# aymenboudhina/Multimodal_VQVAE_compression_audio_tactile

Measured on AMD Instinct MI355X. Metric: encode+VQ+decode token-frames/sec (1 frame = 13.33 ms of paired 24 kHz audio+tactile), higher is better.
Workload: dtype f32

## Files before the change

include/mvq.h:

```cpp
#ifndef MVQ_H
#define MVQ_H

#include <stddef.h>
#include <stdint.h>

#ifdef __cplusplus
extern "C" {
#endif

#define MVQ_OK 0
#define MVQ_EINVAL (-1)
#define MVQ_EUNSUPPORTED (-2)
#define MVQ_EHIP (-3)

#define MVQ_ACT_NONE 0
#define MVQ_ACT_TANH 1
#define MVQ_ACT_GELU 2

int mvq_abi_version(void);
const char* mvq_last_error(void);
unsigned mvq_build_flags(void);

typedef struct mvq_profile_entry {
    char kernel[96];
// ... 305 lines not shown
int mvq_encoder_stream_fwd_f32(const mvq_stack* s, float* state, const int32_t* slots, int n_group, int n_slots, const float* x_new, int n,
                               long long samples_before, int last, float* z, int z_len, void* workspace, size_t workspace_bytes, void* stream);
int mvq_decoder_out_len(const mvq_stack* s, int t);
size_t mvq_decoder_workspace_bytes(const mvq_stack* s, int batch, int t);
int mvq_decoder_fwd_f32(const mvq_stack* s, const float* z, float* y, void* workspace, size_t workspace_bytes, int batch, int t, void* stream);
int mvq_decoder_stream_plan(const mvq_stack* s, int tokens_before, int n, int last, int32_t* stages, int stages_cap, int32_t* emit);
size_t mvq_decoder_stream_state_floats(const mvq_stack* s);
size_t mvq_decoder_stream_workspace_bytes(const mvq_stack* s, int n_group, int tokens_before, int n, int last);
int mvq_decoder_stream_fwd_f32(const mvq_stack* s, float* state, const int32_t* slots, int n_group, int n_slots, const float* z_new, int n,
                               int tokens_before, int last, float* y, int y_len, void* workspace, size_t workspace_bytes, void* stream);
size_t mvq_decoder_saved_bytes(const mvq_stack* s, int batch, int t);
int mvq_decoder_fwd_saving_f32(const mvq_stack* s, const float* z, float* y, void* saved, size_t saved_bytes, void* workspace, size_t workspace_bytes,
                               int batch, int t, void* stream);
int mvq_decoder_bwd_input_f32(const mvq_stack* s, const void* saved, size_t saved_bytes, const float* gy, float* gz, void* workspace,
                              size_t workspace_bytes, int batch, int t, void* stream);

typedef struct mvq_ar_args {
    int batch, t_lat, t_audio, tactile_only, books_use, rvq_k, c_lat, c_ff, code_dim, heads, chunk;
    float ln_eps, tok_eps, scale;
    const float *zt, *k_all, *v_all, *pe;
    const float *lnq_g, *lnq_b, *wq, *wo, *lnf_g, *lnf_b, *w1, *b1, *w3, *b3;
    const float *tok_g, *tok_b, *wd, *bd, *wu, *bu, *books;
    float *z_run, *r_tokens;
    int32_t* idx_out;
} mvq_ar_args;
size_t mvq_ar_workspace_bytes(int batch, int t_lat);
int mvq_ar_latents_f32(const mvq_ar_args* args, void* workspace, size_t workspace_bytes, void* stream);
int mvq_ar_latents_staged_f32(const mvq_ar_args* args, void* workspace, size_t workspace_bytes, void* stream);
int mvq_ar_latents_staged_carry_f32(const mvq_ar_args* args, const float* z_prev, float* z_last_out, void* workspace,
                                    size_t workspace_bytes, void* stream);
int mvq_ar_latents_staged_rate_f32(const mvq_ar_args* args, int packet_tok, int min_books, int mode, float tol2, int budget,
                                   const float* z_prev, float* z_last_out, uint8_t* nb_valid_out, uint8_t* nb_sent_out, void* workspace,
                                   size_t workspace_bytes, void* stream);
int mvq_ar_check(const void* workspace, void* stream);

#ifdef __cplusplus
}
#endif
#endif
```

multimodal_vqvae_compression_audio_tactile_amd/_lib.py:

```python
from __future__ import annotations

import ctypes
import subprocess
from ctypes import c_char_p, c_float, c_int, c_size_t, c_void_p
from pathlib import Path

_PKG = Path(__file__).resolve().parent
import os as _os
SO_PATH = Path(_os.environ["MVQ_LIB_PATH"]).resolve() if _os.environ.get("MVQ_LIB_PATH") else _PKG / "libmvq_hip.so"
_lib = None

class EncoderDesc(ctypes.Structure):
    _fields_ = [("d_model", c_int), ("n_strides", c_int), ("strides", c_int * 8), ("d_latent", c_int)]


class DecoderDesc(ctypes.Structure):
    _fields_ = [("input_channel", c_int), ("channels", c_int), ("n_rates", c_int), ("rates", c_int * 8), ("d_out", c_int), ("output_padding", c_int)]


class ArArgs(ctypes.Structure):
    _fields_ = ([(n, c_int) for n in ("batch", "t_lat", "t_audio", "tactile_only", "books_use", "rvq_k", "c_lat", "c_ff", "code_dim", "heads", "chunk")]
                + [(n, c_float) for n in ("ln_eps", "tok_eps", "scale")]
                + [(n, c_void_p) for n in ("zt", "k_all", "v_all", "pe", "lnq_g", "lnq_b", "wq", "wo", "lnf_g", "lnf_b", "w1", "b1", "w3", "b3",
                                           "tok_g", "tok_b", "wd", "bd", "wu", "bu", "books", "z_run", "r_tokens", "idx_out")])
# ... 123 lines not shown
    "mvq_sub3d_f32": (c_int, [c_void_p, c_size_t, c_size_t] * 3 + [c_int] * 3 + [c_void_p]),
    "mvq_copy3d_f32": (c_int, [c_void_p, c_size_t, c_size_t] * 2 + [c_int] * 3 + [c_void_p]),
    "mvq_encoder_create": (c_int, [ctypes.POINTER(c_void_p), ctypes.POINTER(EncoderDesc), ctypes.POINTER(c_void_p), c_void_p, c_size_t, c_void_p]),
    "mvq_decoder_create": (c_int, [ctypes.POINTER(c_void_p), ctypes.POINTER(DecoderDesc), ctypes.POINTER(c_void_p), c_void_p, c_size_t, c_void_p]),
    "mvq_stack_destroy": (None, [c_void_p]),
    "mvq_stack_param_count": (c_int, [c_void_p]),
    "mvq_stack_param_info": (c_int, [c_void_p, c_int, c_char_p, c_int, ctypes.POINTER(c_int)]),
    "mvq_stack_weights_bytes": (c_size_t, [c_void_p]),
    "mvq_stack_set_plan": (c_int, [c_void_p, c_int, c_int]),
    "mvq_encoder_out_len": (c_int, [c_void_p, c_int]),
    "mvq_encoder_workspace_bytes": (c_size_t, [c_void_p, c_int, c_int]),
    "mvq_encoder_fwd_f32": (c_int, [c_void_p, c_void_p, c_void_p, c_void_p, c_size_t, c_int, c_int, c_void_p]),
    "mvq_decoder_out_len": (c_int, [c_void_p, c_int]),
    "mvq_decoder_workspace_bytes": (c_size_t, [c_void_p, c_int, c_int]),
    "mvq_decoder_fwd_f32": (c_int, [c_void_p, c_void_p, c_void_p, c_void_p, c_size_t, c_int, c_int, c_void_p]),
    "mvq_encoder_stream_plan": (c_int, [c_void_p, ctypes.c_longlong, c_int, c_int, c_void_p, c_int, c_void_p]),
    "mvq_encoder_stream_state_floats": (c_size_t, [c_void_p]),
    "mvq_encoder_stream_workspace_bytes": (c_size_t, [c_void_p, c_int, ctypes.c_longlong, c_int, c_int]),
    "mvq_encoder_stream_fwd_f32": (c_int, [c_void_p, c_void_p, c_void_p, c_int, c_int, c_void_p, c_int, ctypes.c_longlong, c_int, c_void_p, c_int,
                                           c_void_p, c_size_t, c_void_p]),
    "mvq_decoder_stream_plan":(c_int, [c_void_p, c_int, c_int, c_int, c_void_p, c_int, c_void_p]),
    "mvq_decoder_stream_state_floats": (c_size_t, [c_void_p]),
    "mvq_decoder_stream_workspace_bytes": (c_size_t, [c_void_p] + [c_int] * 4),
    "mvq_decoder_stream_fwd_f32": (c_int, [c_void_p, c_void_p, c_void_p, c_int, c_int, c_void_p, c_int, c_int, c_int, c_void_p, c_int, c_void_p,
                                           c_size_t, c_void_p]),
    "mvq_decoder_saved_bytes": (c_size_t, [c_void_p, c_int, c_int]),
    "mvq_decoder_fwd_saving_f32": (c_int, [c_void_p, c_void_p, c_void_p, c_void_p, c_size_t, c_void_p, c_size_t, c_int, c_int, c_void_p]),
    "mvq_decoder_bwd_input_f32": (c_int, [c_void_p, c_void_p, c_size_t, c_void_p, c_void_p, c_void_p, c_size_t, c_int, c_int, c_void_p]),
    "mvq_ar_workspace_bytes": (c_size_t, [c_int, c_int]),
    "mvq_ar_latents_f32": (c_int, [ctypes.POINTER(ArArgs), c_void_p, c_size_t, c_void_p]),
    "mvq_ar_latents_staged_f32": (c_int, [ctypes.POINTER(ArArgs), c_void_p, c_size_t, c_void_p]),
    "mvq_ar_latents_staged_carry_f32": (c_int, [ctypes.POINTER(ArArgs), c_void_p, c_void_p, c_void_p, c_size_t, c_void_p]),
    "mvq_ar_latents_staged_rate_f32": (c_int, [ctypes.POINTER(ArArgs)] + [c_int] * 3 + [c_float, c_int] + [c_void_p] * 5 + [c_size_t, c_void_p]),
    "mvq_ar_check": (c_int, [c_void_p, c_void_p]),
}


class MvqError(RuntimeError):
    """Raised when a libmvq_hip entry point returns a negative status."""


def build(force: bool = False) -> Path:
    args = ["make", "-C", str(_PKG / "csrc"), "-j8"]
    if force:
        args.append("-B")
    res = subprocess.run(args, capture_output=True, text=True)
    if res.returncode != 0:
        raise RuntimeError("building libmvq_hip.so failed:\n" + res.stdout[-4000:] + res.stderr[-4000:])
    return SO_PATH


def lib():
    global _lib
    if _lib is None:
        if not SO_PATH.exists():
            raise MvqError(f"{SO_PATH} is missing: run `python -c 'import __graft_entry__ as g; g.build()'` "
                           "(there is no CPU fallback for the MI355X path)")
        handle = ctypes.CDLL(str(SO_PATH))
        for name, (res, args) in EXPORTS.items():
            fn = getattr(handle, name)
            fn.restype = res
            fn.argtypes = args
        flags = int(handle.mvq_build_flags())
        if flags & 0xFFFF and _os.environ.get("MVQ_ALLOW_TIMING_BUILD") != "1":
            raise MvqError(f"{SO_PATH}: mvq_build_flags() = {flags:#x} (MVQ_NO_DMA in the environment; include/mvq.h).  "
                           "Only A/B runs may load it: set MVQ_ALLOW_TIMING_BUILD=1 to do so.")
# ... 15 lines not shown
```

multimodal_vqvae_compression_audio_tactile_amd/csrc/ar_fused.hip:

```cpp
#include <hip/hip_runtime.h>
#include <stdint.h>
#include <stdio.h>
#include <stdlib.h>
#include "../../include/mvq.h"
#include "conv_dispatch.hpp"
#include "conv_lat.hpp"
#include "kernels_small.hpp"
#include "det_math.hpp"
#include "ln_lat.hpp"

namespace mvq {
void set_last_error(const char* msg);
hipError_t launch_layernorm_lat_io(const LnIo& io, int B, int C, int n, hipStream_t s);

namespace {

constexpr int NTHR = 512;
constexpr int C_LAT = 1024, C_FF = 2048, D_CODE = 96, HEADS = 8, DH = C_LAT / HEADS, CHUNK = 16;

struct ArK {
    mvq_ar_args a;
    float *q16, *qT, *Q16, *ctx16, *y1T, *hdn16, *h16, *zpT, *rN16, *rD16, *qD16;
    unsigned* bar;
    int nblocks;
// ... 307 lines not shown
    if (!a.tactile_only) {
        {
            LnIo& io = tab[0].ln; tab[0].type = ST_LN; tab[0].adv = ADV_LN_PREV | ADV_LN_Y1;
            io.x = nullptr; io.prev = a.z_run; io.prev_sb = cT; io.prev_sc = (size_t)Tl;
            io.pe = a.pe; io.gamma = a.lnq_g; io.beta = a.lnq_b; io.eps = a.ln_eps; io.post_scale = 1.0f;
            io.y0 = k.q16; io.y0_sb = c16; io.y0_sc = p16;
            io.y1 = k.qT; io.y1_sb = cT; io.y1_sc = (size_t)Tl;
        }
        gemm(1, ST_GEMM64, k.q16, C_LAT, a.wq, nullptr, C_LAT, nullptr, 0, k.Q16, CHUNK, 0);
        tab[2].type = ST_ATTN;
        gemm(3, ST_GEMM64, k.ctx16, C_LAT, a.wo, nullptr, C_LAT, k.qT, 0, k.y1T, Tl, ADV_RES | ADV_Y);
        {
            LnIo& io = tab[4].ln; tab[4].type = ST_LN; tab[4].adv = ADV_LN_X;
            io.x = k.y1T; io.x_sb = cT; io.x_sc = (size_t)Tl;
            io.gamma = a.lnf_g; io.beta = a.lnf_b; io.eps = a.ln_eps; io.post_scale = 1.0f;
            io.y0 = k.hdn16; io.y0_sb = c16; io.y0_sc = p16;
        }
        gemm(5, ST_GEMM64, k.hdn16, C_LAT, a.w1, a.b1, C_FF, nullptr, MVQ_ACT_GELU, k.h16, CHUNK, 0);
        gemm(6, ST_GEMM64, k.h16, C_FF, a.w3, a.b3, C_LAT, k.y1T, 0, k.zpT, Tl, ADV_RES | ADV_Y);
        zpred = k.zpT;
    }
    {
        LnIo& io = tab[7].ln; tab[7].type = ST_LN; tab[7].adv = ADV_LN_X | ADV_LN_SUB;
        io.x = a.zt; io.x_sb = cT; io.x_sc = (size_t)Tl;
        io.sub = zpred; io.sub_sb = cT; io.sub_sc = (size_t)Tl;
        io.gamma = a.tok_g; io.beta = a.tok_b; io.eps = a.tok_eps; io.post_scale = a.scale; io.do_tanh = 1;
        io.y0 = k.rN16; io.y0_sb = c16; io.y0_sc = p16;
    }
    gemm(8, ST_GEMM64, k.rN16, C_LAT, a.wd, a.bd, D_CODE, nullptr, 0, k.rD16, CHUNK, 0);
    tab[9].type = ST_RVQ;
    gemm(10, ST_GEMM32, k.qD16, D_CODE, a.wu, a.bu, C_LAT, zpred, 0, a.z_run, Tl, ADV_RES | ADV_Y);
}

}
}

extern "C" {

size_t mvq_ar_workspace_bytes(int batch, int t_lat)
{
    if (batch <= 0 || t_lat <= 0) return 0;
    const size_t c = mvq::C_LAT, p = mvq::CHUNK;
    const size_t f16 = (size_t)batch * p, fT = (size_t)batch * t_lat;
    const size_t floats = c * f16 * 5  + (size_t)mvq::C_FF * f16 + 2 * (size_t)mvq::D_CODE * f16 + c * fT * 3 ;
    return floats * sizeof(float) + 256  + 256 ;
}

static int ar_prepare(const mvq_ar_args* args, void* workspace, size_t workspace_bytes, mvq::ArKT& kt, bool& done)
{
    using namespace mvq;
    auto fail = [](int code, const char* msg) { set_last_error(msg); return code; };
    done = false;
    if (!args) return fail(MVQ_EINVAL, "ar_latents: null argument");
    const mvq_ar_args& a = *args;
    if (a.batch < 0 || a.t_lat < 0 || a.t_audio < 0 || a.books_use < 0) return fail(MVQ_EINVAL, "ar_latents: bad shape");
    if (a.batch == 0 || a.t_lat == 0) { done = true; return MVQ_OK; }
    if (a.c_lat != C_LAT || a.c_ff != C_FF || a.code_dim != D_CODE || a.heads != HEADS || a.chunk != CHUNK)
        return fail(MVQ_EUNSUPPORTED, "ar_latents: the fused loop covers the reference's shapes (c_lat 1024, FFN 2048, 8 heads, code dim 96, chunks of 16)");
    if (a.rvq_k <= 0 || a.rvq_k > 512) return fail(MVQ_EUNSUPPORTED, "ar_latents: K <= 512 codes per book");
    if (!a.zt || !a.z_run || !a.tok_g || !a.tok_b || !a.wd || !a.bd || !a.wu || !a.bu || (a.books_use > 0 && !a.books) || !workspace)
        return fail(MVQ_EINVAL, "ar_latents: null tensor");
    if (!a.tactile_only && (!a.pe || !a.lnq_g || !a.lnq_b || !a.wq || !a.wo || !a.lnf_g || !a.lnf_b || !a.w1 || !a.b1 || !a.w3 || !a.b3 ||
                            (a.t_audio > 0 && (!a.k_all || !a.v_all))))
        return fail(MVQ_EINVAL, "ar_latents: null predictor tensor");
    if (workspace_bytes < mvq_ar_workspace_bytes(a.batch, a.t_lat)) return fail(MVQ_EINVAL, "ar_latents: workspace too small (mvq_ar_workspace_bytes)");
    if ((reinterpret_cast<uintptr_t>(a.books) & 15) != 0) return fail(MVQ_EINVAL, "ar_latents: books must be 16-byte aligned");
    if (conv_mpad(C_LAT) != C_LAT || conv_mpad(C_FF) != C_FF || conv_mpad(D_CODE) != D_CODE) return fail(MVQ_EUNSUPPORTED, "ar_latents: packed-row padding");

    kt = ArKT{};
    ArK& k = kt.k;
    k.a = a;
    char* p = reinterpret_cast<char*>(workspace);
    p += (256 - reinterpret_cast<uintptr_t>(p) % 256) % 256;
    k.bar = reinterpret_cast<unsigned*>(p); p += 256;
    auto take = [&](size_t floats) { float* q = reinterpret_cast<float*>(p); p += floats * sizeof(float); return q; };
    const size_t f16 = (size_t)a.batch * CHUNK, fT = (size_t)a.batch * a.t_lat;
    k.q16 = take(C_LAT * f16); k.Q16 = take(C_LAT * f16); k.ctx16 = take(C_LAT * f16); k.hdn16 = take(C_LAT * f16); k.rN16 = take(C_LAT * f16);
    k.h16 = take((size_t)C_FF * f16); k.rD16 = take((size_t)D_CODE * f16); k.qD16 = take((size_t)D_CODE * f16);
// ... 125 lines not shown
                                             reinterpret_cast<float*>(a.idx_out) + s, (size_t)Tl, 0, a.books_use * B, 1, n, st);
                    if (e == hipSuccess && a.r_tokens)
                        e = launch_strided3d(k.rD16, (size_t)D_CODE * CHUNK, CHUNK, nullptr, 0, 0, a.r_tokens + s, (size_t)D_CODE * Tl, (size_t)Tl, B, D_CODE, n, st);
                    break;
                }
            }
        }
    }
    if (e == hipSuccess && z_last_out)
        e = launch_strided3d(a.z_run + (Tl - 1), (size_t)C_LAT * Tl, (size_t)Tl, nullptr, 0, 0, z_last_out, C_LAT, 1, B, C_LAT, 1, st);
    if (e != hipSuccess) return fail(MVQ_EHIP, hipGetErrorString(e));
    return MVQ_OK;
}

int mvq_ar_latents_staged_f32(const mvq_ar_args* args, void* workspace, size_t workspace_bytes, void* stream)
{
    return ar_staged(args, nullptr, nullptr, workspace, workspace_bytes, stream);
}

int mvq_ar_latents_staged_carry_f32(const mvq_ar_args* args, const float* z_prev, float* z_last_out, void* workspace,
                                    size_t workspace_bytes, void* stream)
{
    return ar_staged(args, z_prev, z_last_out, workspace, workspace_bytes, stream);
}

int mvq_ar_latents_staged_rate_f32(const mvq_ar_args* args, int packet_tok, int min_books, int mode, float tol2, int budget,
                                   const float* z_prev, float* z_last_out, uint8_t* nb_valid_out, uint8_t* nb_sent_out, void* workspace,
                                   size_t workspace_bytes, void* stream)
{
    const ArRate r{packet_tok, min_books, mode, budget, tol2, nb_valid_out, nb_sent_out};
    return ar_staged(args, z_prev, z_last_out, workspace, workspace_bytes, stream, &r);
}

int mvq_ar_check(const void* workspace, void* stream)
{
    if (!workspace) return MVQ_EINVAL;
    const char* p = reinterpret_cast<const char*>(workspace);
    p += (256 - reinterpret_cast<uintptr_t>(p) % 256) % 256;
    unsigned host[2] = {0, 0};
    if (hipMemcpyAsync(host, p, sizeof(host), hipMemcpyDeviceToHost, reinterpret_cast<hipStream_t>(stream)) != hipSuccess) return MVQ_EHIP;
    if (hipStreamSynchronize(reinterpret_cast<hipStream_t>(stream)) != hipSuccess) return MVQ_EHIP;
    if (host[1] != 0) { mvq::set_last_error("ar_latents: a grid barrier gave up (the grid was not co-resident)"); return MVQ_EHIP; }
    return MVQ_OK;
}

}
```

multimodal_vqvae_compression_audio_tactile_amd/csrc/kernels_vq.hip:

```cpp
#include <hip/hip_runtime.h>
#include <stdio.h>
#include <stdint.h>
#include <stdlib.h>
#include <type_traits>
#include "det_math.hpp"
#include "kernels_small.hpp"
#include "dac_stage.hpp"

namespace mvq {

__device__ __forceinline__ void amax_combine(float& s, int& i, float os, int oi)
{
    if (os > s || (os == s && oi < i)) { s = os; i = oi; }
}

__device__ __forceinline__ void wave_argmax(float& s, int& i)
{
#pragma unroll
    for (int off = 32; off >= 1; off >>= 1) {
        const float os = __shfl_xor(s, off);
        const int oi = __shfl_xor(i, off);
        amax_combine(s, i, os, oi);
    }
}
// ... 485 lines not shown
            const float sc = dot - 0.5f * hs;
            if (sc > bs) { bs = sc; bi = tid; }
        }
        wave_argmax(bs, bi);
        if (lane == 0) { ws[wave] = bs; wi[wave] = bi; }
        __syncthreads();
        float cs = ws[0]; int id = wi[0];
#pragma unroll
        for (int w = 1; w < 8; ++w) amax_combine(cs, id, ws[w], wi[w]);
        if (id < 0 || id >= K) id = 0;
        if (tid == id) {
#pragma unroll
            for (int u = 0; u < HV; ++u) *reinterpret_cast<v4*>(qrow + 4 * u) = e0[u];
        }
        if (tid >= 64 && tid < 64 + 4 * HV) qrow[4 * HV + tid - 64] = rows[id * PITCH + tid - 64];
        __syncthreads();
        if (tid < D) {
            const float q = qrow[tid];
            const float r = res[tid];
            qs[tid] = (qs[tid] + (q - r)) + r;
            if (update_residual) res[tid] = r - q;
        }
        if (idx_out && tid == 0) idx_out[(size_t)bk * N + n] = id;
    }
    __syncthreads();
    if (q_out && tid < D) q_out[((size_t)b * D + tid) * T + t] = qs[tid];
}

hipError_t launch_rvq_ema_forward(const float* z, const float* books, float* q_out, int32_t* idx_out,
                                  int B, int D, int T, int nb, int K, int update_residual, hipStream_t s)
{
    const int N = B * T;
    if (N == 0) return hipSuccess;
    if (N <= 256 && D == 96 && K <= 512 && (reinterpret_cast<uintptr_t>(books) & 15) == 0) {
        auto kern = rvq_ema_forward_rows_kernel<24>;
        static BigLdsOptIn opt;
        if (hipError_t e = opt.ensure(reinterpret_cast<const void*>(kern)); e != hipSuccess) return e;
        hipLaunchKernelGGL(kern, dim3(N), dim3(512), ((size_t)K * 52 + 3 * 96 + 16) * sizeof(float), s, z, books, q_out, idx_out, B, T, nb, K, update_residual);
        return hipGetLastError();
    }
    if (N <= 256 && D % 4 == 0 && D <= 128) {
        hipLaunchKernelGGL(rvq_ema_forward_token_kernel, dim3(N), dim3(256), 0, s, z, books, q_out, idx_out, B, D, T, nb, K, update_residual);
        return hipGetLastError();
    }
    const size_t lds_mfma = ((size_t)RVQ_KH * (D + 1) + RVQ_KH + 2 * (size_t)D * 32 + 8 * 32 + 2 * 32) * sizeof(float);
    if (N >= 1024 && D % 4 == 0 && K % 32 == 0 && lds_mfma <= 160 * 1024)
        return launch_rvq_mfma(z, books, q_out, idx_out, B, D, T, nb, K, update_residual, s);
    return N >= 4096 ? launch_rvq_t<32>(z, books, q_out, idx_out, B, D, T, nb, K, update_residual, s)
                     : launch_rvq_t<8>(z, books, q_out, idx_out, B, D, T, nb, K, update_residual, s);
}

constexpr int EMA_SEG = 1024;

__global__ void ema_rows_kernel(const float* __restrict__ z, float* __restrict__ X, int D, int T)
{
    __shared__ float tile[32][33];
    const int b = blockIdx.z, t0 = blockIdx.x * 32, d0 = blockIdx.y * 32;
    const int tx = threadIdx.x & 31, ty = threadIdx.x >> 5;
    for (int r = ty; r < 32; r += 8) {
        const int d = d0 + r, t = t0 + tx;
        tile[r][tx] = (d < D && t < T) ? z[((size_t)b * D + d) * T + t] : 0.0f;
    }
    __syncthreads();
    for (int r = ty; r < 32; r += 8) {
        const int t = t0 + r, d = d0 + tx;
        if (t < T && d < D) X[((size_t)b * T + t) * D + d] = tile[tx][r];
    }
// ... 627 lines not shown
```

multimodal_vqvae_compression_audio_tactile_amd/ops.py:

```python
from __future__ import annotations

import ctypes
import operator

import torch

from . import _lib
from ._lib import MvqError, check
from .stream import resample_stream_out_len


def _stream():
    return torch.cuda.current_stream().cuda_stream


def _dev(t: torch.Tensor, name: str) -> torch.Tensor:
    if not isinstance(t, torch.Tensor):
        raise TypeError(f"{name}: expected a torch.Tensor")
    if t.device.type != "cuda":
        raise MvqError(f"{name}: tensor is on {t.device}; the MI355X path has no CPU fallback")
    if t.dtype != torch.float32:
        t = t.float()
    return t.contiguous()

# ... 888 lines not shown
    if mode not in SSIM_MODES:
        raise MvqError(f"mel_ssim: mode {mode!r} is not one of {sorted(SSIM_MODES)}")
    if not 0 <= int(max_width) <= min(MEL_SSIM_MAX_WIDTH, mel.shape[1]):
        raise MvqError(f"mel_ssim: max_width = {max_width} outside [0, min({MEL_SSIM_MAX_WIDTH}, ld = {mel.shape[1]})]")
    for t, name in ((desc, "desc"), (widths, "widths")) + (((cols, "cols"),) if cols is not None else ()):
        if not isinstance(t, torch.Tensor) or t.device != mel.device or t.dtype != torch.int32:
            raise MvqError(f"mel_ssim: {name} must be an int32 tensor on the device of mel")
    desc, widths = desc.contiguous(), widths.contiguous()
    n = widths.numel()
    if tuple(desc.shape) != (n, 5):
        raise MvqError(f"mel_ssim: desc must be [N = {n}, 5], got {tuple(desc.shape)}")
    cols = cols.contiguous() if cols is not None else None
    out = torch.empty(n, device=mel.device, dtype=torch.float64)
    check(_lib.lib().mvq_mel_ssim_f32(mel.data_ptr(), mel.shape[0], mel.stride(0), maxv.data_ptr(), maxv.numel(), desc.data_ptr(),
                                      _p(cols), 0 if cols is None else cols.numel(), widths.data_ptr(), n, int(max_width),
                                      SSIM_MODES[mode], out.data_ptr(), _stream()), "mvq_mel_ssim_f32")
    return out


def subset_stats(ref, est, latent_mask):
    ref = _dev(ref, "ref").reshape(-1); est = _dev(est, "est").reshape(-1)
    if ref.numel() != est.numel():
        raise MvqError("subset_stats: ref and est must have the same length")
    m = _u8_vec(latent_mask, "subset_stats")
    out = torch.empty(8, device=ref.device, dtype=torch.float64)
    check(_lib.lib().mvq_subset_stats_f32(ref.data_ptr(), est.data_ptr(), ref.numel(), _p(m) if m.numel() else None, m.numel(),
                                          out.data_ptr(), _stream()), "mvq_subset_stats_f32")
    return out


_AR_CHECKED = set()


def ar_latents_fused(zt, z_run, *, k_all, v_all, t_audio, pe, ln_q, wq, wo, ln_f, w1, b1, w3, b3, ln_eps, tok, tok_eps, scale,
                     wd, bd, wu, bu, books, books_use, heads, c_ff, code_dim, r_tokens=None, idx_out=None, tactile_only=False, chunk=16,
                     staged=False, z_prev=None, z_last_out=None, rate=None):
    carried = z_prev is not None or z_last_out is not None
    if rate is not None and (not staged or idx_out is None):
        raise MvqError("ar_latents_fused: rate needs staged=True and idx_out (the persistent kernel has no rate stage)")
    if carried and not staged:
        raise MvqError("ar_latents_fused: z_prev / z_last_out need staged=True (the persistent kernel carries no token)")
    zt = _dev(zt, "zt")
    B, C, Tl = zt.shape
    nb_all, K = (books.shape[0], books.shape[1]) if books is not None else (0, 1)
    nb = nb_all if books_use is None else max(0, min(int(books_use), nb_all))
    a = _lib.ArArgs()
    a.batch, a.t_lat, a.t_audio, a.tactile_only, a.books_use, a.rvq_k = B, Tl, int(t_audio), int(bool(tactile_only)), nb, K
    a.c_lat, a.c_ff, a.code_dim, a.heads, a.chunk = C, int(c_ff), int(code_dim), int(heads), int(chunk)
    a.ln_eps, a.tok_eps, a.scale = float(ln_eps), float(tok_eps), float(scale)
    a.zt, a.z_run, a.r_tokens, a.idx_out = zt.data_ptr(), z_run.data_ptr(), _p(r_tokens), _p(idx_out)
    a.k_all, a.v_all, a.pe = _p(k_all), _p(v_all), _p(pe)
    (a.lnq_g, a.lnq_b), (a.lnf_g, a.lnf_b), (a.tok_g, a.tok_b) = map(lambda t: (_p(t[0]), _p(t[1])), (ln_q, ln_f, tok))
    a.wq, a.wo, a.w1, a.b1, a.w3, a.b3 = _p(wq), _p(wo), _p(w1), _p(b1), _p(w3), _p(b3)
    a.wd, a.bd, a.wu, a.bu, a.books = _p(wd), _p(bd), _p(wu), _p(bu), _p(books)
    L = _lib.lib()
    nbytes = L.mvq_ar_workspace_bytes(B, Tl)
    ws = torch.empty(max(nbytes, 4), device=zt.device, dtype=torch.uint8)
    if rate is not None:
        packet_tok, min_books, mode, tol2, budget, nbv, nbs = rate
        check(L.mvq_ar_latents_staged_rate_f32(ctypes.byref(a), int(packet_tok), int(min_books), int(mode), float(tol2), int(budget),
                                               _p(z_prev), _p(z_last_out), nbv.data_ptr(), nbs.data_ptr(), ws.data_ptr(), nbytes,
                                               _stream()), "mvq_ar_latents_staged_rate_f32")
        return z_run
    if carried:
        check(L.mvq_ar_latents_staged_carry_f32(ctypes.byref(a), _p(z_prev), _p(z_last_out), ws.data_ptr(), nbytes, _stream()),
              "mvq_ar_latents_staged_carry_f32")
        return z_run
    if staged:
        check(L.mvq_ar_latents_staged_f32(ctypes.byref(a), ws.data_ptr(), nbytes, _stream()), "mvq_ar_latents_staged_f32")
        return z_run
    check(L.mvq_ar_latents_f32(ctypes.byref(a), ws.data_ptr(), nbytes, _stream()), "mvq_ar_latents_f32")
    key = (B, Tl, zt.device.index, bool(tactile_only))
    if key not in _AR_CHECKED:
        check(L.mvq_ar_check(ws.data_ptr(), _stream()), "mvq_ar_check")
        _AR_CHECKED.add(key)
    return z_run


def gelu(x):
    x = _dev(x, "x")
    y = torch.empty_like(x)
    check(_lib.lib().mvq_gelu_f32(x.data_ptr(), y.data_ptr(), x.numel(), _stream()), "mvq_gelu_f32")
    return y


def fold_time_slice(a, s, e):
    a = _dev(a, "a")
    B, C, T = a.shape
    n = e - s
    y = torch.empty(1, C, B * n, device=a.device, dtype=torch.float32)
    check(_lib.lib().mvq_copy3d_f32(a.data_ptr() + 4 * s, C * T, T, y.data_ptr(), n, B * n, B, C, n, _stream()),
          "mvq_copy3d_f32")
    return y


# ... 783 lines not shown
```

multimodal_vqvae_compression_audio_tactile_amd/proposed.py:

```python
from __future__ import annotations

import math
import os
from typing import Optional

import numpy as np
import torch
import torch.nn as nn

from . import ops, train
from ._lib import MvqError
from . import dac as _dac
from .dac import _Packed

CODE_DIM = 96
AR_CHUNK_TOK = 16
EMA_DECAY = 0.99


class PosEnc1D(nn.Module):
    def __init__(self, c, max_len=8192):
        super().__init__()
        pe = torch.zeros(max_len, c)
        pos = torch.arange(0, max_len).unsqueeze(1)
# ... 311 lines not shown
                    z_pred = self.predict.run(zt_prev, None, folded_batch=B, kv_all=kv_all, kv_slice=(s, ka))
                else:
                    z_pred = self.predict.run(zt_prev, torch.zeros(1, C, 0, device=zt.device), folded_batch=B)
            rN = ops.layernorm_c(zt_c, ln.weight.detach(), ln.bias.detach(), eps=ln.eps, do_tanh=True, post_scale=scale,
                                 folded_batch=B, sub=z_pred)
            rD = self._pd(rN)
            if books is None:
                qD = torch.zeros_like(rD)
            elif rate is not None:
                _, idx = ops.rvq_ema_forward(rD, books, books_use, return_indices="int32")
                idx_all.append(idx.reshape(idx.shape[0], B, n))
                qD = ops.rvq_rate(rD, idx, books, rate, packet_tok, books_use, folded_batch=B, nb_valid_out=nb_valid,
                                  nb_sent_out=nb_sent, col=s)[0]
            elif want_indices:
                qD, idx = ops.rvq_ema_forward(rD, books, books_use, return_indices=True)
                idx_all.append(idx.reshape(idx.shape[0], B, n))
            else:
                qD = ops.rvq_ema_forward(rD, books, books_use)
            z_hat = self._pu(qD, residual=z_pred)
            ops.unfold_into_(z_run, s, z_hat, B)
            if want_tokens:
                ops.unfold_into_(r_tokens, s, rD, B)
        if z_last_out is not None:
            ops.copy_strided_(z_last_out, 0, (C, 1), z_run, Tlat - 1, (C * Tlat, Tlat), B, C, 1)
        if want_indices:
            idx = torch.cat(idx_all, dim=2).long() if idx_all else torch.zeros(0, B, Tlat, dtype=torch.int64)
            return (z_run, r_tokens, idx) if rate is None else (z_run, r_tokens, idx, nb_valid, nb_sent)
        return z_run, r_tokens

    AR_FUSED_MAX_BATCH = int(_dac.HOST_ENV_SEEN.get("MVQ_AR_FUSED_MAX_BATCH", "0"))

    AR_STAGED_MAX_BATCH = min(8, int(_dac.HOST_ENV_SEEN.get("MVQ_AR_STAGED_MAX_BATCH", "8")))

    def _ar_shapes_covered(self, zt, books):
        p = self.predict
        return (zt.is_cuda and zt.shape[0] > 0 and ops.get_arith() == "f32"
                and zt.shape[1] == 1024 and p.h == 8 and p.ffn[1].out_features == 2048 and CODE_DIM == 96 and p.ln_q.eps == p.ffn[0].eps
                and (books is None or (books.shape[1] <= 512 and books.shape[2] == CODE_DIM)))

    def _ar_one_call_mode(self, zt, books):
        if self._ar_fused_wanted(zt, books):
            return "fused"
        if zt.shape[0] <= self.AR_STAGED_MAX_BATCH and self._ar_shapes_covered(zt, books):
            return "staged"
        return None

    def _ar_fused_wanted(self, zt, books):
        p = self.predict
        return (zt.is_cuda and 0 < zt.shape[0] <= self.AR_FUSED_MAX_BATCH and ops.get_arith() == "f32"
                and not torch.cuda.is_current_stream_capturing()
                and zt.shape[1] == 1024 and p.h == 8 and p.ffn[1].out_features == 2048 and CODE_DIM == 96 and p.ln_q.eps == p.ffn[0].eps
                and (books is None or (books.shape[1] <= 512 and books.shape[2] == CODE_DIM)))

    def _ar_latents_fused(self, zt, z_run, r_tokens, kv_all, t_audio, books, books_use, tactile_only, want_indices, staged=False,
                          z_prev=None, z_last_out=None, rate=None):
        B, _, Tlat = zt.shape
        p, L, ln = self.predict, self.predict._lin, self.tokennorm.ln
        nb = 0 if books is None else (books.shape[0] if books_use is None else max(0, min(int(books_use), books.shape[0])))
        idx = torch.empty(nb, B, Tlat, device=zt.device, dtype=torch.int32) if want_indices else None
        det = lambda t: None if t is None else t.detach()
        ops.ar_latents_fused(
            zt.contiguous(), z_run, k_all=None if kv_all is None else kv_all[0], v_all=None if kv_all is None else kv_all[1],
            t_audio=t_audio if kv_all is not None else 0, pe=p.pos.pe, ln_q=(det(p.ln_q.weight), det(p.ln_q.bias)),
            wq=L["q"].wp(), wo=L["o"].wp(), ln_f=(det(p.ffn[0].weight), det(p.ffn[0].bias)), w1=L["f1"].wp(), b1=det(p.ffn[1].bias),
            w3=L["f3"].wp(), b3=det(p.ffn[3].bias), ln_eps=p.ln_q.eps, tok=(det(ln.weight), det(ln.bias)), tok_eps=ln.eps,
            scale=self._scale_value(), wd=self._pd.wp(), bd=det(self.proj_down.bias), wu=self._pu.wp(), bu=det(self.proj_up.bias),
            books=books, books_use=books_use, heads=p.h, c_ff=p.ffn[1].out_features, code_dim=CODE_DIM, r_tokens=r_tokens, idx_out=idx,
            tactile_only=tactile_only, chunk=AR_CHUNK_TOK, staged=staged, z_prev=z_prev, z_last_out=z_last_out, rate=rate)
        if rate is not None:
            return z_run, r_tokens, idx.long(), rate[5], rate[6]
        if want_indices:
            return z_run, r_tokens, idx.long()
        return z_run, r_tokens

    TWO_STREAM_MAX_BATCH = int(_dac.HOST_ENV_SEEN.get("MVQ_TWO_STREAM_MAX_BATCH", "64"))

    def _encode_branches(self, a_1T, t_1T):
        if a_1T.shape[0] > self.TWO_STREAM_MAX_BATCH or not a_1T.is_cuda or ops.get_arith() != "f32":
            za = self.A_ENC(a_1T)
            qa, *_ = self.A_QUANT(za)
            return qa, self.T_ENC(t_1T)
        cur = torch.cuda.current_stream()
        side = getattr(self, "_side_stream", None)
        if side is None or side.device != a_1T.device:
            side = torch.cuda.Stream(device=a_1T.device)
            self._side_stream = side
        side.wait_stream(cur)
        with torch.cuda.stream(side):
            za = self.A_ENC(a_1T)
            qa, *_ = self.A_QUANT(za)
        zt = self.T_ENC(t_1T)
        cur.wait_stream(side)
        for x in (za, qa):
            x.record_stream(cur)
        return qa, zt

    @torch.no_grad()
    def encode_latents_with_indices(self, a_1T, t_1T, books_use=None, rate=None, packet_tok=None, audio_books=None, audio_rate=None):
        audio = audio_books is not None or audio_rate is not None
        if audio:
            from . import packets
# ... 623 lines not shown
```

Before: 61740.

## Add two-pass AR latent path batching all chunks in one pass

Adds a two-pass autoregressive latent routine. Pass one runs every prediction stage over all chunks at once as wide GEMMs. A second pass then recomputes only the first token of each chunk, using the previous chunk's last output, and scatters the results back. This replaces the per-chunk sequential staged loop with a few large launches, cutting kernel-launch count and serialization at the cost of extra workspace and redundant compute. The RVQ rows-kernel threshold is also widened so the larger column counts use the LDS-resident path.

```diff
diff --git a/include/mvq.h b/include/mvq.h
--- a/include/mvq.h
+++ b/include/mvq.h
@@ -361,6 +361,9 @@
 int mvq_ar_latents_staged_rate_f32(const mvq_ar_args* args, int packet_tok, int min_books, int mode, float tol2, int budget,
                                    const float* z_prev, float* z_last_out, uint8_t* nb_valid_out, uint8_t* nb_sent_out, void* workspace,
                                    size_t workspace_bytes, void* stream);
+int mvq_ar_two_pass_wanted(int batch, int t_lat, int tactile_only, int carried);
+int mvq_ar_latents_two_pass_f32(const mvq_ar_args* args, const float* z_prev, float* z_last_out, void* workspace,
+                                size_t workspace_bytes, void* stream);
 int mvq_ar_check(const void* workspace, void* stream);
 
 #ifdef __cplusplus
diff --git a/multimodal_vqvae_compression_audio_tactile_amd/_lib.py b/multimodal_vqvae_compression_audio_tactile_amd/_lib.py
--- a/multimodal_vqvae_compression_audio_tactile_amd/_lib.py
+++ b/multimodal_vqvae_compression_audio_tactile_amd/_lib.py
@@ -179,6 +179,8 @@
     "mvq_ar_latents_staged_f32": (c_int, [ctypes.POINTER(ArArgs), c_void_p, c_size_t, c_void_p]),
     "mvq_ar_latents_staged_carry_f32": (c_int, [ctypes.POINTER(ArArgs), c_void_p, c_void_p, c_void_p, c_size_t, c_void_p]),
     "mvq_ar_latents_staged_rate_f32": (c_int, [ctypes.POINTER(ArArgs)] + [c_int] * 3 + [c_float, c_int] + [c_void_p] * 5 + [c_size_t, c_void_p]),
+    "mvq_ar_two_pass_wanted": (c_int, [c_int] * 4),
+    "mvq_ar_latents_two_pass_f32": (c_int, [ctypes.POINTER(ArArgs), c_void_p, c_void_p, c_void_p, c_size_t, c_void_p]),
     "mvq_ar_check": (c_int, [c_void_p, c_void_p]),
 }
 
diff --git a/multimodal_vqvae_compression_audio_tactile_amd/csrc/ar_fused.hip b/multimodal_vqvae_compression_audio_tactile_amd/csrc/ar_fused.hip
--- a/multimodal_vqvae_compression_audio_tactile_amd/csrc/ar_fused.hip
+++ b/multimodal_vqvae_compression_audio_tactile_amd/csrc/ar_fused.hip
@@ -363,6 +363,22 @@
     gemm(10, ST_GEMM32, k.qD16, D_CODE, a.wu, a.bu, C_LAT, zpred, 0, a.z_run, Tl, ADV_RES | ADV_Y);
 }
 
+struct TwoPassDims { int NC, P, G; size_t N; };
+inline TwoPassDims two_pass_dims(int batch, int t_lat)
+{
+    TwoPassDims d;
+    d.NC = (t_lat + CHUNK - 1) / CHUNK; d.P = d.NC * CHUNK; d.G = batch * d.NC; d.N = (size_t)batch * d.P;
+    return d;
+}
+constexpr int TP_N_BUFS = 12, TP_G_BUFS = 10;
+inline size_t tp_round(size_t floats) { return (floats + 63) & ~(size_t)63; }
+inline size_t two_pass_floats(int batch, int t_lat)
+{
+    const TwoPassDims d = two_pass_dims(batch, t_lat);
+    return TP_N_BUFS * tp_round(C_LAT * d.N) + tp_round(C_FF * d.N) + 2 * tp_round(D_CODE * d.N) +
+           TP_G_BUFS * tp_round((size_t)C_LAT * d.G) + tp_round((size_t)C_FF * d.G) + 2 * tp_round((size_t)D_CODE * d.G);
+}
+
 }
 }
 
@@ -374,7 +390,9 @@
     const size_t c = mvq::C_LAT, p = mvq::CHUNK;
     const size_t f16 = (size_t)batch * p, fT = (size_t)batch * t_lat;
     const size_t floats = c * f16 * 5  + (size_t)mvq::C_FF * f16 + 2 * (size_t)mvq::D_CODE * f16 + c * fT * 3 ;
-    return floats * sizeof(float) + 256  + 256 ;
+    const size_t chunk_plan = floats * sizeof(float) + 256  + 256 ;
+    const size_t two_pass = mvq::two_pass_floats(batch, t_lat) * sizeof(float) + 256 ;
+    return chunk_plan > two_pass ? chunk_plan : two_pass;
 }
 
 static int ar_prepare(const mvq_ar_args* args, void* workspace, size_t workspace_bytes, mvq::ArKT& kt, bool& done)
@@ -566,6 +584,172 @@
     return ar_staged(args, z_prev, z_last_out, workspace, workspace_bytes, stream, &r);
 }
 
+}
+
+namespace mvq {
+namespace {
+
+__global__ void ar_gather2_kernel(const float* __restrict__ z_run, const float* __restrict__ zt, const float* __restrict__ z_prev,
+                                  float* __restrict__ x2, float* __restrict__ zt2, int B, int NC, int Tl)
+{
+    const int G = B * NC;
+    const size_t total = (size_t)C_LAT * G;
+    for (size_t e = blockIdx.x * (size_t)blockDim.x + threadIdx.x; e < total; e += (size_t)gridDim.x * blockDim.x) {
+        const int ch = (int)(e / G), g = (int)(e - (size_t)ch * G);
+        const int b = g / NC, c = g - b * NC;
+        const size_t row = ((size_t)b * C_LAT + ch) * Tl;
+        x2[e] = c > 0 ? z_run[row + (size_t)c * CHUNK - 1] : (z_prev ? z_prev[(size_t)b * C_LAT + ch] : 0.0f);
+        zt2[e] = zt[row + (size_t)c * CHUNK];
+    }
+}
+
+__global__ void ar_scatter2_kernel(const float* __restrict__ z2, const float* __restrict__ rD2, const int32_t* __restrict__ idx2,
+                                   float* __restrict__ z_run, float* __restrict__ r_tokens, int32_t* __restrict__ idx_out,
+                                   int B, int NC, int Tl, int nb)
+{
+    const int G = B * NC;
+    const size_t nz = (size_t)C_LAT * G, nr = r_tokens ? (size_t)D_CODE * G : 0, ni = idx_out ? (size_t)nb * G : 0;
+    for (size_t e = blockIdx.x * (size_t)blockDim.x + threadIdx.x; e < nz + nr + ni; e += (size_t)gridDim.x * blockDim.x) {
+        const size_t r = e < nz ? e : (e < nz + nr ? e - nz : e - nz - nr);
+        const int row = (int)(r / G), g = (int)(r - (size_t)row * G);
+        const int b = g / NC, c = g - b * NC;
+        const size_t col = (size_t)c * CHUNK;
+        if (e < nz) z_run[((size_t)b * C_LAT + row) * Tl + col] = z2[r];
+        else if (e < nz + nr) r_tokens[((size_t)b * D_CODE + row) * Tl + col] = rD2[r];
+        else idx_out[((size_t)row * B + b) * Tl + col] = idx2[r];
+    }
+}
+
+struct TpCols { float *x, *zt, *q, *Q, *ctx, *y1, *hdn, *h, *zp, *rN, *rD, *qD, *z; };
+
+}
+}
+
+extern "C" {
+
+int mvq_ar_two_pass_wanted(int batch, int t_lat, int tactile_only, int carried)
+{
+    if (batch <= 0 || t_lat <= 0 || (tactile_only && carried)) return 0;
+    const int nc = (t_lat + mvq::CHUNK - 1) / mvq::CHUNK;
+    return tactile_only ? nc >= 2 : nc >= 3;
+}
+
+int mvq_ar_latents_two_pass_f32(const mvq_ar_args* args, const float* z_prev, float* z_last_out, void* workspace, size_t workspace_bytes,
+                                void* stream)
+{
+    using namespace mvq;
+    auto fail = [](int code, const char* msg) { set_last_error(msg); return code; };
+    ArKT kt;
+    bool done = false;
+    if (const int rc = ar_prepare(args, workspace, workspace_bytes, kt, done); rc != MVQ_OK || done) return rc;
+    const mvq_ar_args& a = kt.k.a;
+    if ((z_prev || z_last_out) && a.tactile_only) return fail(MVQ_EINVAL, "ar_latents_two_pass: tactile_only has no recursion to carry");
+    if (a.books_use > C_LAT) return fail(MVQ_EUNSUPPORTED, "ar_latents_two_pass: too many books");
+    hipStream_t st = reinterpret_cast<hipStream_t>(stream);
+    const int B = a.batch, Tl = a.t_lat, nb = a.books_use;
+    const TwoPassDims dm = two_pass_dims(B, Tl);
+    const int NC = dm.NC, P = dm.P, G = dm.G;
+    const size_t N = dm.N;
+    if (N > 0x7fffffffu / 4) return fail(MVQ_EUNSUPPORTED, "ar_latents_two_pass: sequence too long");
+    const int Ta = a.tactile_only ? 0 : (a.t_audio < Tl ? a.t_audio : Tl);
+    const int nfull = Ta / CHUNK;
+    const bool pass2 = !a.tactile_only && (NC > 1 || z_prev);
+    const bool kv_direct = B == 1 || Ta == P;
+    const bool kv_padded = !kv_direct && nfull > 0;
+
+    char* p = reinterpret_cast<char*>(workspace);
+    p += (256 - reinterpret_cast<uintptr_t>(p) % 256) % 256;
+    auto take = [&](size_t floats) { float* q = reinterpret_cast<float*>(p); p += tp_round(floats) * sizeof(float); return q; };
+    TpCols c1{}, c2{};
+    c1.x = take(C_LAT * N); c1.zt = take(C_LAT * N); c1.ctx = take(C_LAT * N);
+    float* const Kp = take(C_LAT * N);
+    float* const Vp = take(C_LAT * N);
+    c1.q = take(C_LAT * N); c1.Q = take(C_LAT * N); c1.y1 = take(C_LAT * N); c1.hdn = take(C_LAT * N);
+    c1.zp = take(C_LAT * N); c1.rN = take(C_LAT * N); c1.z = take(C_LAT * N);
+    c1.h = take(C_FF * N); c1.rD = take(D_CODE * N); c1.qD = take(D_CODE * N);
+    const size_t cg = (size_t)C_LAT * G;
+    c2.x = take(cg); c2.zt = take(cg); c2.q = take(cg); c2.Q = take(cg); c2.ctx = take(cg); c2.y1 = take(cg); c2.hdn = take(cg);
+    c2.zp = take(cg); c2.rN = take(cg); c2.z = take(cg);
+    c2.h = take((size_t)C_FF * G); c2.rD = take((size_t)D_CODE * G); c2.qD = take((size_t)D_CODE * G);
+
+    int rc = MVQ_OK;
+    auto hip = [&](hipError_t e) { if (rc == MVQ_OK && e != hipSuccess) rc = fail(MVQ_EHIP, hipGetErrorString(e)); };
+    auto api = [&](int r) { if (rc == MVQ_OK && r != MVQ_OK) rc = r; };
+    auto zero = [&](float* ptr, size_t floats) {
+        if (rc != MVQ_OK) return;
+        const size_t n4 = tp_round(floats) / 4;
+        size_t blocks = (n4 + 255) / 256; if (blocks > 1024) blocks = 1024;
+        hipLaunchKernelGGL(ar_zero_kernel, dim3((unsigned)blocks), dim3(256), 0, st, reinterpret_cast<float4*>(ptr), n4);
+        hip(hipGetLastError());
+    };
+    auto gemm = [&](const float* x, int cin, const float* wp, const float* bias, int cout, const float* res, int act, float* y, size_t cols) {
+        if (rc == MVQ_OK) api(mvq_conv1d_f32(x, wp, bias, nullptr, res, nullptr, y, 1, cin, (int)cols, cout, 1, 1, 1, 0, act, stream));
+    };
+    auto ln = [&](const float* x, const float* sub, const float* pe, const float* g, const float* bt, float* y, int groups, int t, size_t cols,
+                  float eps, int do_tanh, float post) {
+        if (rc == MVQ_OK) api(mvq_layernorm_c_sub_f32(x, sub, pe, g, bt, y, groups, C_LAT, t, (size_t)t, cols, eps, do_tanh, post, stream));
+    };
+    auto stages = [&](const TpCols& c, int t, size_t cols, int32_t* idx) {
+        const float* zpred = nullptr;
+        if (!a.tactile_only) {
+            ln(c.x, nullptr, a.pe, a.lnq_g, a.lnq_b, c.q, G, t, cols, a.ln_eps, 0, 1.0f);
+            gemm(c.q, C_LAT, a.wq, nullptr, C_LAT, nullptr, 0, c.Q, cols);
+            if (rc == MVQ_OK && nfull > 0)
+                api(mvq_attention_f32(c.Q, kv_padded ? Kp : a.k_all, kv_padded ? Vp : a.v_all, c.ctx, kv_padded || Ta == P ? G : nfull, HEADS, DH,
+                                      t, CHUNK, (size_t)t, cols, CHUNK, kv_padded ? N : (size_t)B * Ta, stream));
+            for (int ch = nfull; ch < NC && rc == MVQ_OK; ++ch) {
+                const int s = ch * CHUNK, nt = Tl - s < CHUNK ? Tl - s : CHUNK;
+                const int ka = (Ta < s + nt ? Ta : s + nt) - (Ta < s ? Ta : s);
+                const float* kc = ka > 0 ? a.k_all + s : c.Q;
+                const float* vc = ka > 0 ? a.v_all + s : c.Q;
+                api(mvq_attention_f32(c.Q + (size_t)ch * t, kc, vc, c.ctx + (size_t)ch * t, B, HEADS, DH, t < nt ? t : nt, ka, (size_t)NC * t, cols,
+                                      (size_t)Ta, (size_t)B * Ta, stream));
+            }
+            gemm(c.ctx, C_LAT, a.wo, nullptr, C_LAT, c.q, 0, c.y1, cols);
+            ln(c.y1, nullptr, nullptr, a.lnf_g, a.lnf_b, c.hdn, G, t, cols, a.ln_eps, 0, 1.0f);
+            gemm(c.hdn, C_LAT, a.w1, a.b1, C_FF, nullptr, MVQ_ACT_GELU, c.h, cols);
+            gemm(c.h, C_FF, a.w3, a.b3, C_LAT, c.y1, 0, c.zp, cols);
+            zpred = c.zp;
+        }
+        ln(c.zt, zpred, nullptr, a.tok_g, a.tok_b, c.rN, G, t, cols, a.tok_eps, 1, a.scale);
+        gemm(c.rN, C_LAT, a.wd, a.bd, D_CODE, nullptr, 0, c.rD, cols);
+        if (nb > 0) {
+            if (rc == MVQ_OK) hip(launch_rvq_ema_forward(c.rD, a.books, c.qD, a.idx_out ? idx : nullptr, 1, D_CODE, (int)cols, nb, a.rvq_k, 1, st));
+        } else zero(c.qD, D_CODE * cols);
+        gemm(c.qD, D_CODE, a.wu, a.bu, C_LAT, zpred, 0, c.z, cols);
+    };
+
+    zero(c1.x, (kv_padded ? 5 : 3) * tp_round(C_LAT * N));
+    if (rc == MVQ_OK) hip(launch_strided3d(a.zt, (size_t)C_LAT * Tl, (size_t)Tl, nullptr, 0, 0, c1.zt, (size_t)P, N, B, C_LAT, Tl, st));
+    if (kv_padded && rc == MVQ_OK) {
+        hip(launch_strided3d(a.k_all, (size_t)Ta, (size_t)B * Ta, nullptr, 0, 0, Kp, (size_t)P, N, B, C_LAT, Ta, st));
+        if (rc == MVQ_OK) hip(launch_strided3d(a.v_all, (size_t)Ta, (size_t)B * Ta, nullptr, 0, 0, Vp, (size_t)P, N, B, C_LAT, Ta, st));
+    }
+    int32_t* const idx1 = reinterpret_cast<int32_t*>(c1.ctx);
+    stages(c1, CHUNK, N, idx1);
+    if (rc == MVQ_OK) hip(launch_strided3d(c1.z, (size_t)P, N, nullptr, 0, 0, a.z_run, (size_t)C_LAT * Tl, (size_t)Tl, B, C_LAT, Tl, st));
+    if (rc == MVQ_OK && a.r_tokens)
+        hip(launch_strided3d(c1.rD, (size_t)P, N, nullptr, 0, 0, a.r_tokens, (size_t)D_CODE * Tl, (size_t)Tl, B, D_CODE, Tl, st));
+    if (rc == MVQ_OK && a.idx_out && nb > 0)
+        hip(launch_strided3d(reinterpret_cast<const float*>(idx1), (size_t)P, 0, nullptr, 0, 0, reinterpret_cast<float*>(a.idx_out), (size_t)Tl, 0,
+                             nb * B, 1, Tl, st));
+    if (pass2 && rc == MVQ_OK) {
+        size_t blocks = ((size_t)C_LAT * G + 255) / 256; if (blocks > 1024) blocks = 1024;
+        hipLaunchKernelGGL(ar_gather2_kernel, dim3((unsigned)blocks), dim3(256), 0, st, a.z_run, a.zt, z_prev, c2.x, c2.zt, B, NC, Tl);
+        hip(hipGetLastError());
+        int32_t* const idx2 = reinterpret_cast<int32_t*>(c2.ctx);
+        stages(c2, 1, (size_t)G, idx2);
+        if (rc == MVQ_OK) {
+            hipLaunchKernelGGL(ar_scatter2_kernel, dim3((unsigned)blocks), dim3(256), 0, st, c2.z, c2.rD, idx2, a.z_run, a.r_tokens,
+                               nb > 0 ? a.idx_out : nullptr, B, NC, Tl, nb);
+            hip(hipGetLastError());
+        }
+    }
+    if (rc == MVQ_OK && z_last_out)
+        hip(launch_strided3d(a.z_run + (Tl - 1), (size_t)C_LAT * Tl, (size_t)Tl, nullptr, 0, 0, z_last_out, C_LAT, 1, B, C_LAT, 1, st));
+    return rc;
+}
+
 int mvq_ar_check(const void* workspace, void* stream)
 {
     if (!workspace) return MVQ_EINVAL;
diff --git a/multimodal_vqvae_compression_audio_tactile_amd/csrc/kernels_vq.hip b/multimodal_vqvae_compression_audio_tactile_amd/csrc/kernels_vq.hip
--- a/multimodal_vqvae_compression_audio_tactile_amd/csrc/kernels_vq.hip
+++ b/multimodal_vqvae_compression_audio_tactile_amd/csrc/kernels_vq.hip
@@ -541,7 +541,7 @@
 {
     const int N = B * T;
     if (N == 0) return hipSuccess;
-    if (N <= 256 && D == 96 && K <= 512 && (reinterpret_cast<uintptr_t>(books) & 15) == 0) {
+    if (N < 1024 && D == 96 && K <= 512 && (reinterpret_cast<uintptr_t>(books) & 15) == 0) {
         auto kern = rvq_ema_forward_rows_kernel<24>;
         static BigLdsOptIn opt;
         if (hipError_t e = opt.ensure(reinterpret_cast<const void*>(kern)); e != hipSuccess) return e;
diff --git a/multimodal_vqvae_compression_audio_tactile_amd/ops.py b/multimodal_vqvae_compression_audio_tactile_amd/ops.py
--- a/multimodal_vqvae_compression_audio_tactile_amd/ops.py
+++ b/multimodal_vqvae_compression_audio_tactile_amd/ops.py
@@ -944,9 +944,15 @@
 _AR_CHECKED = set()
 
 
+def ar_two_pass_taken(batch, t_lat, tactile_only=False, carried=False, rate=None, two_pass=True) -> bool:
+    if not two_pass or rate is not None or get_arith() != "f32" or (tactile_only and carried):
+        return False
+    return two_pass == "force" or bool(_lib.lib().mvq_ar_two_pass_wanted(int(batch), int(t_lat), int(bool(tactile_only)), int(bool(carried))))
+
+
 def ar_latents_fused(zt, z_run, *, k_all, v_all, t_audio, pe, ln_q, wq, wo, ln_f, w1, b1, w3, b3, ln_eps, tok, tok_eps, scale,
                      wd, bd, wu, bu, books, books_use, heads, c_ff, code_dim, r_tokens=None, idx_out=None, tactile_only=False, chunk=16,
-                     staged=False, z_prev=None, z_last_out=None, rate=None):
+                     staged=False, z_prev=None, z_last_out=None, rate=None, two_pass=False):
     carried = z_prev is not None or z_last_out is not None
     if rate is not None and (not staged or idx_out is None):
         raise MvqError("ar_latents_fused: rate needs staged=True and idx_out (the persistent kernel has no rate stage)")
@@ -973,6 +979,10 @@
         check(L.mvq_ar_latents_staged_rate_f32(ctypes.byref(a), int(packet_tok), int(min_books), int(mode), float(tol2), int(budget),
                                                _p(z_prev), _p(z_last_out), nbv.data_ptr(), nbs.data_ptr(), ws.data_ptr(), nbytes,
                                                _stream()), "mvq_ar_latents_staged_rate_f32")
+        return z_run
+    if staged and ar_two_pass_taken(B, Tl, tactile_only, carried, rate, two_pass):
+        check(L.mvq_ar_latents_two_pass_f32(ctypes.byref(a), _p(z_prev), _p(z_last_out), ws.data_ptr(), nbytes, _stream()),
+              "mvq_ar_latents_two_pass_f32")
         return z_run
     if carried:
         check(L.mvq_ar_latents_staged_carry_f32(ctypes.byref(a), _p(z_prev), _p(z_last_out), ws.data_ptr(), nbytes, _stream()),
diff --git a/multimodal_vqvae_compression_audio_tactile_amd/proposed.py b/multimodal_vqvae_compression_audio_tactile_amd/proposed.py
--- a/multimodal_vqvae_compression_audio_tactile_amd/proposed.py
+++ b/multimodal_vqvae_compression_audio_tactile_amd/proposed.py
@@ -367,6 +367,8 @@
 
     AR_STAGED_MAX_BATCH = min(8, int(_dac.HOST_ENV_SEEN.get("MVQ_AR_STAGED_MAX_BATCH", "8")))
 
+    AR_TWO_PASS = True
+
     def _ar_shapes_covered(self, zt, books):
         p = self.predict
         return (zt.is_cuda and zt.shape[0] > 0 and ops.get_arith() == "f32"
@@ -401,7 +403,8 @@
             w3=L["f3"].wp(), b3=det(p.ffn[3].bias), ln_eps=p.ln_q.eps, tok=(det(ln.weight), det(ln.bias)), tok_eps=ln.eps,
             scale=self._scale_value(), wd=self._pd.wp(), bd=det(self.proj_down.bias), wu=self._pu.wp(), bu=det(self.proj_up.bias),
             books=books, books_use=books_use, heads=p.h, c_ff=p.ffn[1].out_features, code_dim=CODE_DIM, r_tokens=r_tokens, idx_out=idx,
-            tactile_only=tactile_only, chunk=AR_CHUNK_TOK, staged=staged, z_prev=z_prev, z_last_out=z_last_out, rate=rate)
+            tactile_only=tactile_only, chunk=AR_CHUNK_TOK, staged=staged, z_prev=z_prev, z_last_out=z_last_out, rate=rate,
+            two_pass=self.AR_TWO_PASS if staged and rate is None else False)
         if rate is not None:
             return z_run, r_tokens, idx.long(), rate[5], rate[6]
         if want_indices:
```

After: 61730. About the same (-0.0%).
